# data-mermaid/mermaid-classifier

Measured on AMD Instinct MI355X. Metric: patches/sec (224x224 EfficientNet-B0), higher is better.
Workload: dtype f16; 1 GPU; EfficientNet-B0 forward, batch=256 random 224x224 u8 patches per GPU -> (256,1280) fp32; per_gpu_batch=256, global_batch=256, weights=synthetic seed 0, input_batches_rotated=8, lanes_per_gpu=2, parallelism=patch-sharded x1

## Files before the change

### mermaid_classifier_amd/csrc/k_mid.hip

```cpp
#include "device_common.h"

template <int CKS, int KSD, int CE>
__global__ __launch_bounds__(512) void mid14_kernel(Mid14Args a)
{
    constexpr int HW = 196, CH = 96, NCHK = CE / CH, NPF = 13, NTILE = 6 * NPF, NBAND = 5;
    constexpr int ES2 = 416;
    constexpr int R = KSD / 2, NP = KSD == 5 ? 3 : 2;
    static_assert(CE % CH == 0, "chunking");
    extern __shared__ __attribute__((aligned(16))) unsigned char smem[];
    constexpr int ZT = R, ZB = R + 1;
    unsigned char* E = smem + ZT * 7 * ES2;
    float* pband = reinterpret_cast<float*>(smem + (98 + 7 * (ZT + ZB)) * ES2);
    const int tid = threadIdx.x, lane = tid & 63, wave = __builtin_amdgcn_readfirstlane(tid >> 6);
    const int m = lane & 15, q = lane >> 4;
    const int b = blockIdx.x;
    const int Cin = a.Cin;
    const GLOBAL_AS _Float16* wexp = sgpr_ptr<_Float16>(a.wexp);
    const GLOBAL_AS float* bexp = sgpr_ptr<float>(a.bexp);
    const GLOBAL_AS uint32_t* dwp = sgpr_ptr<uint32_t>(a.dwp);
    const GLOBAL_AS float* bdw = sgpr_ptr<float>(a.bdw);
    const int npf = wave < 5 ? 2 : 1;
    const int pf0 = wave < 5 ? 2 * wave : wave + 5;
    const GLOBAL_AS _Float16* xgp = sgpr_ptr<_Float16>(a.X) + (size_t)b * HW * Cin;
    const int band0 = tid / CH, cd = tid - band0 * CH;
// ... 72 lines not shown
#pragma unroll
                        for (int i = 0; i < NPFW; ++i) acc[i] = __builtin_amdgcn_mfma_f32_16x16x32_f16(xb[i][ks], wc[ks], acc[i], 0, 0, 0);
                    float t[4 * NPFW];
#pragma unroll
                    for (int i = 0; i < NPFW; ++i)
#pragma unroll
                        for (int j = 0; j < 4; ++j) t[4 * i + j] = acc[i][j];
                    silu_scaled_staged(t);
#pragma unroll
                    for (int i = 0; i < NPFW; ++i) {
                        const int pix0 = 16 * (pf0 + i) + 4 * q;
                        const h2 p0 = {(_Float16)t[4 * i], (_Float16)t[4 * i + 1]};
                        const h2 p1 = {(_Float16)t[4 * i + 2], (_Float16)t[4 * i + 3]};
                        const bool ok = pix0 < HW;
                        unsigned char* dst = E + (pix0 >> 1) * ES2 + (16 * nf + m) * 4;
                        *reinterpret_cast<h2*>(ok ? dst : scratch) = p0;
                        *reinterpret_cast<h2*>(ok ? dst + ES2 : scratch + 256) = p1;
                    }
                }
            };
            if (npf == 2) expand_chunk(std::integral_constant<int, 2>{});
            else expand_chunk(std::integral_constant<int, 1>{});
        }
        T7_BAR();
        {
            constexpr int NR = 3 + 2 * R;
            const unsigned char* col = E + 4 * cd + ((rb - R) * 7) * ES2;
            uint32_t P[NR][7];
#pragma unroll
            for (int r = 0; r < NR; ++r)
#pragma unroll
                for (int pp = 0; pp < 7; ++pp) P[r][pp] = *reinterpret_cast<const uint32_t*>(col + (r * 7 + pp) * ES2);
            f2 psum2 = {0.f, 0.f};
            uint16_t* dg = reinterpret_cast<uint16_t*>(a.D + (size_t)b * HW * CE + chunk * CH + cd);
#pragma unroll
            for (int ro = 0; ro < 3; ++ro) {
                const int oy = rb + ro;
                if (oy < 14) {
                    float acc[14];
                    bool started[14] = {false, false, false, false, false, false, false, false, false, false, false, false, false, false};
#pragma unroll
                    for (int ky = 0; ky < KSD; ++ky) {
                        const uint32_t r0 = raw[3 * ky], r1 = raw[3 * ky + 1], r2 = raw[3 * ky + 2];
                        uint32_t wq[2][3];
                        if (KSD == 5) {
                            wq[0][0] = r0; wq[0][1] = r1; wq[0][2] = r2;
                            wq[1][0] = r0 << 16; wq[1][1] = __builtin_amdgcn_alignbit(r1, r0, 16); wq[1][2] = __builtin_amdgcn_alignbit(r2, r1, 16);
                        } else {
                            wq[0][0] = r0 << 16; wq[0][1] = __builtin_amdgcn_alignbit(r1, r0, 16); wq[0][2] = 0u;
                            wq[1][0] = r0; wq[1][1] = r1; wq[1][2] = 0u;
                        }
#pragma unroll
                        for (int ip = 0; ip < NP; ++ip)
#pragma unroll
                            for (int ox = 0; ox < 14; ++ox) {
                                const int fp = (KSD == 5 || !(ox & 1)) ? (ox >> 1) - 1 : (ox >> 1);
                                const int xpc = fp + ip;
                                if (xpc < 0 || xpc > 6) continue;
                                if (!started[ox]) { acc[ox] = dot2_from(P[ro + ky][xpc], wq[ox & 1][ip], dbias); started[ox] = true; }
                                else acc[ox] = __builtin_amdgcn_fdot2(*reinterpret_cast<const h2*>(&P[ro + ky][xpc]),
                                                                      *reinterpret_cast<const h2*>(&wq[ox & 1][ip]), acc[ox], false);
                            }
                    }
                    silu_scaled_staged(acc);
#pragma unroll
                    for (int ox = 0; ox < 14; ox += 2) {
                        const f2 v = {acc[ox], acc[ox + 1]};
                        psum2 = psum2 + v;
                        const uint32_t hv = cvt_pk_f16(acc[ox], acc[ox + 1]);
                        dg[(size_t)(oy * 14 + ox) * CE] = (uint16_t)hv;
                        dg[(size_t)(oy * 14 + ox + 1) * CE] = (uint16_t)(hv >> 16);
                    }
                }
            }
            pband[band * CH + cd] = (psum2.x + psum2.y) + 0.f;
        }
        T7_BAR();
        if (tid < CH)
            a.pool[(size_t)b * CE + chunk * CH + tid] =
                ((pband[tid] + pband[CH + tid]) + pband[2 * CH + tid]) + pband[3 * CH + tid] + pband[4 * CH + tid];
    }
}

template <int CKS, int KSD, int CE>
__global__ __launch_bounds__(512) void mid14m_kernel(Mid14Args a)
{
    constexpr int HW = 196, NG = CE / 16, R = KSD / 2;
    constexpr int XSTR = 64 * CKS + 16;
    constexpr int ERS = 40;
    constexpr int ECS = 736;
    constexpr int EREG = 16 * ECS;
    constexpr int TREG = 56 * 32;
    extern __shared__ __attribute__((aligned(16))) unsigned char smem[];
    unsigned char* XS = smem;
    const int tid = threadIdx.x, lane = tid & 63, wave = __builtin_amdgcn_readfirstlane(tid >> 6);
    unsigned char* EW = smem + HW * XSTR + wave * (EREG + TREG);
    unsigned char* TW = EW + EREG;
    const int n16 = lane & 15, q = lane >> 4;
    const int blk = lane >> 2, n = lane & 3;
    const int c = 2 * (blk & 3) + ((blk >> 2) & 1) + 8 * (blk >> 3);
    const int b = blockIdx.x;
    const int Cin = a.Cin;
    const GLOBAL_AS _Float16* wexp = sgpr_ptr<_Float16>(a.wexp);
    const GLOBAL_AS float* bexp = sgpr_ptr<float>(a.bexp);
    const GLOBAL_AS _Float16* dwt = sgpr_ptr<_Float16>(a.dwdiag);
    const GLOBAL_AS float* bdw = sgpr_ptr<float>(a.bdw);
    const bool clk = a.dbg_clk != nullptr;
    long long ck[5] = {clk ? (long long)__builtin_readcyclecounter() : 0, 0, 0, 0, 0};
    {
        const _Float16* xg = a.X + (size_t)b * HW * Cin;
        constexpr int CPR = 4 * CKS;
        constexpr int NIT = (HW * CPR + 511) / 512;
        uint4 xv[NIT];
        for (int e = lane; e < EREG / 16; e += 64) *reinterpret_cast<uint4*>(EW + 16 * e) = uint4{0u, 0u, 0u, 0u};
#pragma unroll
        for (int it = 0; it < NIT; ++it) {
            const int e0 = tid + 512 * it, e = e0 < HW * CPR ? e0 : HW * CPR - 1;
            const int row = e / CPR, cc = e - row * CPR;
            xv[it] = *reinterpret_cast<const uint4*>(xg + (size_t)row * Cin + (8 * cc < Cin ? 8 * cc : Cin - 8));
        }
#pragma unroll
        for (int it = 0; it < NIT; ++it) {
            const int e = tid + 512 * it;
            const int row = e / CPR, cc = e - row * CPR;
            const uint4 v = 8 * cc < Cin ? xv[it] : uint4{0u, 0u, 0u, 0u};
            if (e < HW * CPR) *reinterpret_cast<uint4*>(XS + row * XSTR + 16 * cc) = v;
        }
    }
    __syncthreads();
    if (clk) ck[1] = (long long)__builtin_readcyclecounter();
    const unsigned char* xrow = XS + (n16 < 14 ? n16 : 13) * XSTR + 16 * q;
    unsigned char* est = EW + n16 * ECS + 2 * ERS + 8 * q;
    const uint32_t m3 = q == 3 ? 0u : 0xffffffffu;
    const unsigned char* dld = EW + c * ECS + n * ERS + (2 - R) * ERS;
    const unsigned char* dld3 = EW + c * ECS + (n < 2 ? n : 1) * ERS + (2 - R) * ERS;
    unsigned char* tst = TW + (n * 14 + (((blk >> 2) & 1) ? 7 : 0)) * 32 + (c >> 1) * 4;
    h8 we[CKS], wen[CKS];
    u2v ta[KSD][2], tan[KSD][2];
    float be, bd, ben, bdn;
    auto request_group = [&](int g, h8 (&w1)[CKS], u2v (&w2)[KSD][2], float& b1, float& b2) {
#pragma unroll
        for (int ks = 0; ks < CKS; ++ks) w1[ks] = gload<h8>(wexp, (unsigned)(((g * CKS + ks) * 64 + lane) * 16));
        b1 = gload<float>(bexp, (unsigned)(16 * g + n16) * 4u);
#pragma unroll
        for (int ky = 0; ky < KSD; ++ky)
#pragma unroll
            for (int h = 0; h < 2; ++h) w2[ky][h] = gload<u2v>(dwt, (unsigned)((((g * KSD + ky) * 2 + h) * 64 + lane) * 8));
        b2 = gload<float>(bdw, (unsigned)(16 * g + c) * 4u);
    };
    {
        const int g0 = blockIdx.y * 8 + wave;
        request_group(g0 < NG ? g0 : 0, wen, tan, ben, bdn);
    }
#pragma unroll 1
    for (int g = blockIdx.y * 8 + wave; g < NG; g += 8 * gridDim.y) {
#pragma unroll
        for (int ks = 0; ks < CKS; ++ks) we[ks] = wen[ks];
#pragma unroll
        for (int ky = 0; ky < KSD; ++ky) { ta[ky][0] = tan[ky][0]; ta[ky][1] = tan[ky][1]; }
        be = ben;
        bd = bdn;
        {
            const int gn = g + 8 * (int)gridDim.y;
            request_group(gn < NG ? gn : g, wen, tan, ben, bdn);
        }
        PIN_VMEM();
        auto x_frags = [&](int y, h8 (&xb)[2][CKS]) {
#pragma unroll
            for (int u = 0; u < 2; ++u)
#pragma unroll
                for (int ks = 0; ks < CKS; ++ks) xb[u][ks] = *reinterpret_cast<const h8*>(xrow + (y + u) * 14 * XSTR + 64 * ks);
        };
        auto x_epilogue = [&](int y, const f4 (&acc)[2]) {
            float t[8] = {acc[0][0], acc[0][1], acc[0][2], acc[0][3], acc[1][0], acc[1][1], acc[1][2], acc[1][3]};
            silu_scaled_staged(t);
#pragma unroll
            for (int u = 0; u < 2; ++u) {
                const u2v o = {cvt_pk_f16(t[4 * u], t[4 * u + 1]), cvt_pk_f16(t[4 * u + 2], t[4 * u + 3]) & m3};
                *reinterpret_cast<u2v*>(est + (y + u) * ERS) = o;
            }
        };
        {
            const f4 bev = {be, be, be, be};
            h8 xf[2][2][CKS];
            f4 accp[2] = {bev, bev};
            x_frags(0, xf[0]);
#pragma unroll
            for (int st = 0; st < 7; ++st) {
                if (st + 1 < 7) x_frags(2 * (st + 1), xf[(st + 1) & 1]);
                __builtin_amdgcn_sched_barrier(0);
                f4 acc[2];
#pragma unroll
                for (int ks = 0; ks < CKS; ++ks)
#pragma unroll
                    for (int u = 0; u < 2; ++u)
                        acc[u] = __builtin_amdgcn_mfma_f32_16x16x32_f16(xf[st & 1][u][ks], we[ks], ks == 0 ? bev : acc[u], 0, 0, 0);
                if (st > 0) x_epilogue(2 * (st - 1), accp);
                if (st > 0) {
#pragma unroll
                    for (int i = 0; i < 2 * CKS; ++i) {
                        __builtin_amdgcn_sched_group_barrier(0x008, 1, 0);
                        __builtin_amdgcn_sched_group_barrier(0x002, 5, 0);
                    }
                }
                __builtin_amdgcn_sched_barrier(0);
#pragma unroll
                for (int u = 0; u < 2; ++u) accp[u] = acc[u];
            }
            x_epilogue(12, accp);
        }
        if (clk && ck[2] == 0) ck[2] = (long long)__builtin_readcyclecounter();
        float psum = 0.f;
        unsigned char* dgb = reinterpret_cast<unsigned char*>(a.D + (size_t)b * HW * CE + 16 * g);
        auto d_quads = [&](auto yt_tag, h4 (&bq)[KSD][4]) {
            constexpr int YT = decltype(yt_tag)::value;
            const unsigned char* rb = YT == 3 ? dld3 : dld;
#pragma unroll
            for (int ky = 0; ky < KSD; ++ky)
#pragma unroll
                for (int x4 = 0; x4 < 4; ++x4) bq[ky][x4] = *reinterpret_cast<const h4*>(rb + (4 * YT + ky) * ERS + 8 * x4);
        };
        auto d_strip = [&](const h4 (&bq)[KSD][4], f4 (&acc)[4]) {
            const f4 bdv = {bd, bd, bd, bd};
#pragma unroll
            for (int ky = 0; ky < KSD; ++ky) {
                const h4 a0 = __builtin_bit_cast(h4, ta[ky][0]), a1 = __builtin_bit_cast(h4, ta[ky][1]);
#pragma unroll
                for (int xt = 0; xt < 4; ++xt) acc[xt] = __builtin_amdgcn_mfma_f32_4x4x4f16(a1, bq[ky][xt], ky == 0 ? bdv : acc[xt], 0, 0, 0);
#pragma unroll
                for (int xt = 1; xt < 4; ++xt) acc[xt] = __builtin_amdgcn_mfma_f32_4x4x4f16(a0, bq[ky][xt - 1], acc[xt], 0, 0, 0);
            }
        };
        auto d_epilogue = [&](auto yt_tag, const f4 (&acc)[4]) {
            constexpr int YT = decltype(yt_tag)::value;
            float v[14];
#pragma unroll
            for (int x = 0; x < 14; ++x) v[x] = acc[(x + 2) >> 2][(x + 2) & 3];
            silu_scaled_staged(v);
            float s = ((v[0] + v[1]) + (v[2] + v[3])) + ((v[4] + v[5]) + (v[6] + v[7])) + ((v[8] + v[9]) + (v[10] + v[11])) + (v[12] + v[13]);
            if (YT == 3) s = n < 2 ? s : 0.f;
            psum += s;
#ifdef MID14M_NOSWAP
#pragma unroll
            for (int x = 0; x < 14; x += 2) {
                const uint32_t hv = cvt_pk_f16(v[x], v[x + 1]);
                *reinterpret_cast<uint16_t*>(TW + (n * 14 + x) * 32 + c * 2) = (uint16_t)hv;
                *reinterpret_cast<uint16_t*>(TW + (n * 14 + x + 1) * 32 + c * 2) = (uint16_t)(hv >> 16);
            }
#else
#pragma unroll
            for (int j = 0; j < 7; ++j) {
                float lo = v[j], hi = v[7 + j];
                asm volatile("s_nop 1\n\tv_permlane16_swap_b32 %0, %1\n\ts_nop 1" : "+v"(lo), "+v"(hi));
                *reinterpret_cast<uint32_t*>(tst + j * 32) = cvt_pk_f16(lo, hi);
            }
#endif
            constexpr int NV = YT == 3 ? 56 : 112;
#pragma unroll
            for (int r = 0; r < 2; ++r) {
                if (64 * r >= NV) break;
                const int v0 = lane + 64 * r, vi = v0 < NV ? v0 : NV - 1;
                const uint4 o = *reinterpret_cast<const uint4*>(TW + vi * 16);
                *reinterpret_cast<uint4*>(dgb + (size_t)(56 * YT + (vi >> 1)) * (CE * 2) + 16 * (vi & 1)) = o;
            }
        };
        {
            using I0 = std::integral_constant<int, 0>; using I1 = std::integral_constant<int, 1>;
            using I2 = std::integral_constant<int, 2>; using I3 = std::integral_constant<int, 3>;
            h4 bqa[KSD][4], bqb[KSD][4];
            f4 acc0[4], acc1[4];
            d_quads(I0{}, bqa);
            d_quads(I1{}, bqb);
            __builtin_amdgcn_sched_barrier(0);
            d_strip(bqa, acc0);
            __builtin_amdgcn_sched_barrier(0);
            d_quads(I2{}, bqa);
            __builtin_amdgcn_sched_barrier(0);
            d_strip(bqb, acc1);
            d_epilogue(I0{}, acc0);
            __builtin_amdgcn_sched_barrier(0);
            d_quads(I3{}, bqb);
            __builtin_amdgcn_sched_barrier(0);
            d_strip(bqa, acc0);
            d_epilogue(I1{}, acc1);
            __builtin_amdgcn_sched_barrier(0);
            d_strip(bqb, acc1);
            d_epilogue(I2{}, acc0);
            __builtin_amdgcn_sched_barrier(0);
            d_epilogue(I3{}, acc1);
        }
        psum = quad_sum(psum);
        if (n == 0) a.pool[(size_t)b * CE + 16 * g + c] = psum;
        if (clk && ck[3] == 0) ck[3] = (long long)__builtin_readcyclecounter();
    }
    if (clk && lane == 0 && (wave == 0 || wave == 4 || wave == 7)) {
        ck[4] = (long long)__builtin_readcyclecounter();
        float* dst = a.dbg_clk + ((size_t)b * 8 + blockIdx.y) * 16 + (wave == 0 ? 0 : (wave == 4 ? 4 : 8));
        dst[0] = (float)(ck[1] - ck[0]); dst[1] = (float)(ck[2] - ck[1]); dst[2] = (float)(ck[3] - ck[2]); dst[3] = (float)(ck[4] - ck[3]);
    }
}

template <int KS, int NF, int HW, bool RES>
__global__ __launch_bounds__(512) void proj_patch_kernel(ProjPatchArgs a)
{
    constexpr int CK = (KS <= 8) ? KS : (KS % 7 == 0 ? 3 : (KS % 5 == 0 ? (NF <= 5 ? 3 : 5) : 6));
    constexpr int NCH = KS / CK;
    static_assert(KS % CK == 0, "chunking");
    constexpr int NPF = (HW + 15) / 16, NPAIR = (NPF + 1) / 2;
    constexpr int NWCH = NF * KS * 64;
    constexpr int WPT = (NWCH + 511) / 512;
    constexpr int KP = 32 * KS;
    constexpr bool EARLY_RES = KS < 21;
    extern __shared__ __attribute__((aligned(16))) unsigned char smem[];
    unsigned char* wl = smem;
    float* pooled = reinterpret_cast<float*>(smem + NF * KS * 1024);
    float* gate = pooled + KP;
    float* rs = gate + KP;
    const int tid = threadIdx.x, lane = tid & 63, wave = __builtin_amdgcn_readfirstlane(tid >> 6);
    const int m = lane & 15, q = lane >> 4;
    const int b = blockIdx.x;
    const int K = a.K, CSP = a.CSP;
    long long tk0 = 0, tk1 = 0, tk2 = 0;
    if (a.dbg_clk) tk0 = (long long)__builtin_readcyclecounter();
    const GLOBAL_AS _Float16* wfrag = sgpr_ptr<_Float16>(a.wfrag);
    const GLOBAL_AS _Float16* wr_g = sgpr_ptr<_Float16>(a.wr_g);
    const GLOBAL_AS _Float16* we_t = sgpr_ptr<_Float16>(a.we_t);
    const GLOBAL_AS float* pp = sgpr_ptr<float>(a.pool_part);
    constexpr int FC1_IT = (KP + 63) / 64, KPAD = 64 * FC1_IT;
    const int G = CSP >> 2;
    const bool fc1_wave = wave < G;
    const GLOBAL_AS _Float16* xg = sgpr_ptr<_Float16>(a.X) + (size_t)b * HW * K;
    auto load_chunk = [&](int pr, int ch, h8 (&dst)[2][CK]) {
#pragma unroll
        for (int i = 0; i < 2; ++i) {
            const int p = 32 * pr + 16 * i + m;
            const int pix = p < HW ? p : HW - 1;
#pragma unroll
            for (int u = 0; u < CK; ++u) {
                const int k = 32 * (ch * CK + u) + 8 * q;
                dst[i][u] = gload<h8>(xg, (unsigned)((pix * K + (k < K ? k : K - 8)) * 2));
            }
        }
    };
    constexpr int NW = NF * KS;
    constexpr int DS0 = NW < 44 ? NW : 44, DS1 = NW - DS0 < 50 ? NW - DS0 : 50;
    auto dma = [&](auto i0_tag, auto i1_tag) {
        constexpr int I0 = decltype(i0_tag)::value, I1 = decltype(i1_tag)::value;
#pragma unroll
        for (int i = I0; i < I1; ++i)
            __builtin_amdgcn_global_load_lds((const __attribute__((address_space(1))) void*)(a.wfrag + ((size_t)i * 64 + lane) * 8),
                                             (__attribute__((address_space(3))) void*)(wl + i * 1024), 16, 0, 0);
        PIN_VMEM();
    };
    h8 xc[2][CK], xn[2][CK];
    f4 bv[NF];
    const GLOBAL_AS float* biasg = sgpr_ptr<float>(a.bias);
    auto load_bias = [&]() {
#pragma unroll
        for (int nf = 0; nf < NF; ++nf) bv[nf] = gload<f4>(biasg, (unsigned)(16 * nf + 4 * q) * 4u);
    };
    if (wave == 7) {
        __builtin_amdgcn_s_barrier();
        dma(std::integral_constant<int, 0>{}, std::integral_constant<int, DS0>{});
        T7_BAR();
        dma(std::integral_constant<int, DS0>{}, std::integral_constant<int, DS0 + DS1>{});
        T7_BAR();
        dma(std::integral_constant<int, DS0 + DS1>{}, std::integral_constant<int, NW>{});
        load_bias();
        if (7 < NPAIR) { load_chunk(7, 0, xc); PIN_VMEM(); }
        asm volatile("s_waitcnt vmcnt(0)" ::: "memory");
        T7_BAR();
    } else {
        static_assert(KP <= 672, "channel 448..511 reassignment assumes no channel t + 512 for t >= 160");
        float ps0 = 0.f, ps1 = 0.f;
        const int pk0 = tid, pk1 = (tid >= 160 && tid < 224) ? tid + 288 : tid + 512;
        {
            const int k0 = pk0 < K ? pk0 : 0, k1 = pk1 < K ? pk1 : 0;
            if (a.nparts == 1) {
                ps0 = gload<float>(pp, (unsigned)((b * K + k0) * 4));
                ps1 = gload<float>(pp, (unsigned)((b * K + k1) * 4));
            } else {
                float v0[16], v1[16];
#pragma unroll
                for (int p = 0; p < 16; ++p) {
                    const int pc = p < a.nparts ? p : 0;
                    v0[p] = gload<float>(pp, (unsigned)(((b * a.nparts + pc) * K + k0) * 4));
                    v1[p] = gload<float>(pp, (unsigned)(((b * a.nparts + pc) * K + k1) * 4));
                }
#pragma unroll
                for (int p = 0; p < 16; ++p) {
                    ps0 += p < a.nparts ? v0[p] : 0.f;
                    ps1 += p < a.nparts ? v1[p] : 0.f;
                }
            }
        }
        const int wj = fc1_wave ? wave : 0;
        u2v w1[FC1_IT];
#pragma unroll
        for (int i = 0; i < FC1_IT; ++i) w1[i] = gload<u2v>(wr_g, (unsigned)(((wj * KPAD + lane + 64 * i) * 4) * 2));
        const int k2 = 2 * tid;
        const bool fc2_thr = k2 < K;
        uint32_t w2[28];
#pragma unroll
        for (int j = 0; j < 28; ++j) w2[j] = gload<uint32_t>(we_t, (unsigned)(((j < CSP ? j : 0) * K + (fc2_thr ? k2 : 0)) * 2));
        const float be0 = fc2_thr ? a.be[k2] : 0.f, be1 = fc2_thr ? a.be[k2 + 1] : 0.f;
        load_bias();
        const float brv = a.br[4 * wj + (lane & 3)];
    PIN_VMEM();
    __builtin_amdgcn_s_barrier();
    if (pk0 < KP) pooled[pk0] = pk0 < K ? ps0 : 0.f;
    if (pk1 < KP) pooled[pk1] = pk1 < K ? ps1 : 0.f;
    T7_BAR();
    if (a.dbg_clk && tid == 0) a.dbg_clk[(size_t)b * 8 + 3] = (float)((long long)__builtin_readcyclecounter() - tk0);
    if (fc1_wave) {
        float xs[FC1_IT];
#pragma unroll
        for (int i = 0; i < FC1_IT; ++i) {
            const int k = lane + 64 * i;
            xs[i] = pooled[k < KP ? k : 0];
        }
        __builtin_amdgcn_sched_barrier(0);
        float acc[4] = {0.f, 0.f, 0.f, 0.f};
#pragma unroll
        for (int i = 0; i < FC1_IT; ++i) {
            acc[0] = fma_mix_lo(w1[i].x, xs[i], acc[0]);
            acc[1] = fma_mix_hi(w1[i].x, xs[i], acc[1]);
            acc[2] = fma_mix_lo(w1[i].y, xs[i], acc[2]);
            acc[3] = fma_mix_hi(w1[i].y, xs[i], acc[3]);
        }
        float tot[4];
#pragma unroll
        for (int j = 0; j < 4; ++j) {
            const int v = __builtin_bit_cast(int, row16_sum(acc[j]));
            tot[j] = (__builtin_bit_cast(float, __builtin_amdgcn_readlane(v, 0)) + __builtin_bit_cast(float, __builtin_amdgcn_readlane(v, 16))) +
                     (__builtin_bit_cast(float, __builtin_amdgcn_readlane(v, 32)) + __builtin_bit_cast(float, __builtin_amdgcn_readlane(v, 48)));
        }
        if (lane < 4) {
            const float sv = lane == 0 ? tot[0] : (lane == 1 ? tot[1] : (lane == 2 ? tot[2] : tot[3]));
            rs[4 * wave + lane] = silu_f(sv * a.psc + brv);
        }
    }
    T7_BAR();
    if (a.dbg_clk && tid == 0) {
        a.dbg_clk[(size_t)b * 8 + 4] = (float)((long long)__builtin_readcyclecounter() - tk0);
        a.dbg_clk[(size_t)b * 8 + 5] = a.dbg_clk[(size_t)b * 8 + 4];
    }
    static_assert(NPAIR >= 7, "waves 0..6 all own a pair of pixel fragments");
    load_chunk(wave, 0, xc);
    PIN_VMEM();
    if (k2 < KP) {
        float a0 = be0, a1 = be1;
// ... 200 lines not shown
```

### mermaid_classifier_amd/csrc/k_tail.hip

```cpp
#include "device_common.h"

#define T7_PIX 49
#define T7_C 192
#define T7_CE 1152
#define T7_XS 400
#define T7_ES 2320
#define T7_YS 656
#define T7_DS11 1552
#define T7_OFF_X (T7_PIX * T7_ES)
#define T7_OFF_POOL (T7_OFF_X + T7_PIX * T7_XS)
#define T7_OFF_RS (T7_OFF_POOL + T7_CE * 4)
#define T7_OFF_GATE (T7_OFF_RS + 48 * 4)
#define T7_OFF_PART (T7_OFF_GATE + T7_CE * 4)
#define T7_LDS 163680
static_assert(T7_LDS >= T7_OFF_PART + 32 * 48 * 4 && T7_LDS <= 163840, "tail7 LDS map");

#ifndef T7_GATE_IN_WEIGHTS
#define T7_GATE_IN_WEIGHTS 0
#endif

#define DW_SILU(acc) silu_scaled_staged(acc)
__global__ __launch_bounds__(512) void tail7_kernel(TailArgs a)
{
    extern __shared__ __attribute__((aligned(16))) unsigned char smem[];
// ... 6 lines not shown
    const int tid0 = threadIdx.x;
    const int b = blockIdx.x;
    const bool clk_on = a.dbg_clk && a.clk_sections;
    long long tkk[6] = {0, 0, 0, 0, 0, 0};
    if (clk_on) tkk[0] = (long long)__builtin_readcyclecounter();
    auto proj_prefetch = [&](const GLOBAL_AS _Float16* wproj, const GLOBAL_AS float* bproj, int KS, int nf0, int nfn, int lane, int q,
                             f4 (&pbias)[3], unsigned (&wo)[3], h8 (&wa)[3][4]) {
#pragma unroll
        for (int i = 0; i < 3; ++i) {
            const int nf = nf0 + (i < nfn ? i : 0);
            pbias[i] = gload<f4>(bproj, (unsigned)(16 * nf + 4 * q) * 4u);
            wo[i] = (unsigned)((nf * KS * 64 + lane) * 16);
#pragma unroll
            for (int d = 0; d < 4; ++d) wa[i][d] = gload<h8>(wproj, wo[i] + (unsigned)(d * 1024));
        }
    };
    auto proj_run = [&](const GLOBAL_AS _Float16* wproj, int KS, int mode, int nf0, int nfn, int lane, int m, int q,
                        const int (&pixc)[4], f4 (&pbias)[3], unsigned (&wo)[3], h8 (&wa)[3][4], int es = T7_ES) {
        f4 acc[3][4];
#pragma unroll
        for (int i = 0; i < 3; ++i)
#pragma unroll
            for (int pf = 0; pf < 4; ++pf) acc[i][pf] = pbias[i];
        const unsigned char* bxp[4];
#pragma unroll
        for (int pf = 0; pf < 4; ++pf) bxp[pf] = ED + pixc[pf] * es + 16 * q;
        auto k_loop = [&](auto nf_tag, auto ks_tag) {
            constexpr int NF = decltype(nf_tag)::value, KSC = decltype(ks_tag)::value;
            static_assert(KSC % 4 == 0 && KSC >= 8, "k-steps come in sets of four");
            h8 bx[4], bn[4], wb[NF][4];
#pragma unroll
            for (int pf = 0; pf < 4; ++pf) bx[pf] = *reinterpret_cast<const h8*>(bxp[pf]);
            f4 gc0 = *reinterpret_cast<const f4*>(gate + 8 * q), gc1 = *reinterpret_cast<const f4*>(gate + 8 * q + 4), gn0, gn1;
            auto gated = [&](const h8& w) -> h8 {
                if (!T7_GATE_IN_WEIGHTS) return w;
                const uint4 o = gate_h8(*reinterpret_cast<const uint4*>(&w), gc0, gc1);
                return *reinterpret_cast<const h8*>(&o);
            };
            auto step = [&](int ks, const h8 (&wset)[3][4], int d) {
                const int kn = ks + 1 < KSC ? ks + 1 : KSC - 1;
#pragma unroll
                for (int pf = 0; pf < 4; ++pf) bn[pf] = *reinterpret_cast<const h8*>(bxp[pf] + 64 * kn);
                if (T7_GATE_IN_WEIGHTS) {
                    gn0 = *reinterpret_cast<const f4*>(gate + 32 * kn + 8 * q);
                    gn1 = *reinterpret_cast<const f4*>(gate + 32 * kn + 8 * q + 4);
                }
                h8 wg[NF];
#pragma unroll
                for (int i = 0; i < NF; ++i) wg[i] = gated(wset[i][d]);
#pragma unroll
                for (int i = 0; i < NF; ++i)
#pragma unroll
                    for (int pf = 0; pf < 4; ++pf)
                        acc[i][pf] = __builtin_amdgcn_mfma_f32_16x16x32_f16(wg[i], bx[pf], acc[i][pf], 0, 0, 0);
#pragma unroll
                for (int pf = 0; pf < 4; ++pf) bx[pf] = bn[pf];
                gc0 = gn0; gc1 = gn1;
            };
            auto stepb = [&](int ks, int d) {
                const int kn = ks + 1 < KSC ? ks + 1 : KSC - 1;
#pragma unroll
                for (int pf = 0; pf < 4; ++pf) bn[pf] = *reinterpret_cast<const h8*>(bxp[pf] + 64 * kn);
                if (T7_GATE_IN_WEIGHTS) {
                    gn0 = *reinterpret_cast<const f4*>(gate + 32 * kn + 8 * q);
                    gn1 = *reinterpret_cast<const f4*>(gate + 32 * kn + 8 * q + 4);
                }
                h8 wg[NF];
#pragma unroll
                for (int i = 0; i < NF; ++i) wg[i] = gated(wb[i][d]);
#pragma unroll
                for (int i = 0; i < NF; ++i)
#pragma unroll
                    for (int pf = 0; pf < 4; ++pf)
                        acc[i][pf] = __builtin_amdgcn_mfma_f32_16x16x32_f16(wg[i], bx[pf], acc[i][pf], 0, 0, 0);
#pragma unroll
                for (int pf = 0; pf < 4; ++pf) bx[pf] = bn[pf];
                gc0 = gn0; gc1 = gn1;
            };
#pragma unroll 1
            for (int k0 = 0; k0 + 8 <= KSC; k0 += 8) {
#pragma unroll
                for (int d = 0; d < 4; ++d) {
#pragma unroll
                    for (int i = 0; i < NF; ++i) wb[i][d] = gload<h8>(wproj, wo[i] + (unsigned)((k0 + 4 + d) * 1024));
                    PIN_VMEM();
                    step(k0 + d, wa, d);
                    PIN_VMEM();
                }
#pragma unroll
                for (int d = 0; d < 4; ++d) {
                    const int kw = k0 + 8 + d < KSC ? k0 + 8 + d : KSC - 1;
#pragma unroll
                    for (int i = 0; i < NF; ++i) wa[i][d] = gload<h8>(wproj, wo[i] + (unsigned)(kw * 1024));
                    PIN_VMEM();
                    stepb(k0 + 4 + d, d);
                    PIN_VMEM();
                }
            }
            if (KSC % 8) {
#pragma unroll
                for (int d = 0; d < 4; ++d) step(KSC - 4 + d, wa, d);
            }
        };
        auto run_nf = [&](auto ks_tag) {
            if (nfn == 3) k_loop(std::integral_constant<int, 3>{}, ks_tag);
            else if (nfn == 2) k_loop(std::integral_constant<int, 2>{}, ks_tag);
            else k_loop(std::integral_constant<int, 1>{}, ks_tag);
        };
        if (KS == 36) run_nf(std::integral_constant<int, 36>{});
        else run_nf(std::integral_constant<int, 24>{});
        if (mode == 1) {
            T7_BAR();
#pragma unroll
            for (int pf = 0; pf < 4; ++pf) {
                if (16 * pf + m >= T7_PIX) continue;
#pragma unroll
                for (int i = 0; i < 3; ++i) {
                    if (i >= nfn) continue;
                    h4 o;
#pragma unroll
                    for (int j = 0; j < 4; ++j) o[j] = (_Float16)acc[i][pf][j];
                    *reinterpret_cast<h4*>(ED + (16 * pf + m) * T7_YS + (16 * (nf0 + i) + 4 * q) * 2) = o;
                }
            }
        } else {
#pragma unroll
            for (int pf = 0; pf < 4; ++pf) {
                if (16 * pf + m >= T7_PIX) continue;
#pragma unroll
                for (int i = 0; i < 2; ++i) {
                    if (i >= nfn) continue;
                    h4* px = reinterpret_cast<h4*>(XL + (16 * pf + m) * T7_XS + (16 * (nf0 + i) + 4 * q) * 2);
                    h4 r = {0, 0, 0, 0};
                    if (mode == 0) r = *px;
                    h4 o;
#pragma unroll
                    for (int j = 0; j < 4; ++j) o[j] = (_Float16)(acc[i][pf][j] + (float)r[j]);
                    *px = o;
                }
            }
        }
    };
    if (a.pre_D || a.pre_X) {
        const int DS = a.pre_X ? T7_DS11 : T7_ES;
        const int tid = tid0, lane = tid & 63, wave = __builtin_amdgcn_readfirstlane(tid >> 6);
        const int m = lane & 15, q = lane >> 4;
        const GLOBAL_AS _Float16* wr_t = sgpr_ptr<_Float16>(a.pre_wr_t);
        const GLOBAL_AS _Float16* we_t = sgpr_ptr<_Float16>(a.pre_we_t);
        const GLOBAL_AS _Float16* wproj = sgpr_ptr<_Float16>(a.pre_wproj);
        const GLOBAL_AS float* bproj = sgpr_ptr<float>(a.pre_bproj);
        const int sl = tid / 7, j4 = tid - sl * 7;
        const bool fc_thr = tid < 336;
        u2v w1[14];
#pragma unroll
        for (int i = 0; i < 14; ++i) w1[i] = gload<u2v>(wr_t, (unsigned)((((fc_thr ? sl : 0) + 48 * i) * 28 + 4 * j4) * 2));
        uint32_t w2[28];
#pragma unroll
        for (int j = 0; j < 28; ++j) w2[j] = gload<uint32_t>(we_t, (unsigned)((j * 672 + (fc_thr ? 2 * tid : 0)) * 2));
        const float be0 = fc_thr ? a.pre_be[2 * tid] : 0.f, be1 = fc_thr ? a.pre_be[2 * tid + 1] : 0.f;
        const float brv = tid < 28 ? a.pre_br[tid] : 0.f;
        if (a.pre_X) {
            constexpr int CH = 96, ES2 = 416;
            unsigned char* EB = ED + T7_PIX * T7_DS11 + 7 * ES2;
            float* pband = part;
            const GLOBAL_AS _Float16* wexp = sgpr_ptr<_Float16>(a.pre_wexp);
            const GLOBAL_AS float* bexp = sgpr_ptr<float>(a.pre_bexp);
            const GLOBAL_AS uint32_t* dwp = sgpr_ptr<uint32_t>(a.pre_dwp);
            const GLOBAL_AS float* bdw = sgpr_ptr<float>(a.pre_bdw);
            const GLOBAL_AS _Float16* xgp = sgpr_ptr<_Float16>(a.pre_X) + (size_t)b * 196 * 112;
            const int npf = wave < 5 ? 2 : 1;
            const int pf0 = wave < 5 ? 2 * wave : wave + 5;
            h8 xb[2][4];
#pragma unroll
            for (int i = 0; i < 2; ++i) {
                const int pix = 16 * (pf0 + (i < npf ? i : 0)) + m;
                const int pixc = pix < 196 ? pix : 195;
#pragma unroll
                for (int ks = 0; ks < 4; ++ks) {
                    const int kk = 32 * ks + 8 * q;
                    xb[i][ks] = gload<h8>(xgp, (unsigned)((pixc * 112 + (kk < 112 ? kk : 104)) * 2));
                }
            }
            for (int e = tid; e < T7_PIX * 12; e += 512) {
                const int pix = e / 12, oc = e - pix * 12;
                *reinterpret_cast<uint4*>(ED + pix * T7_DS11 + 1344 + oc * 16) = uint4{0u, 0u, 0u, 0u};
            }
            for (int e = tid; e < 35 * (ES2 / 16); e += 512) {
                const int row = e / (ES2 / 16), c16 = e - row * (ES2 / 16);
                *reinterpret_cast<uint4*>(EB + (row < 7 ? row - 7 : row + 91) * ES2 + 16 * c16) = uint4{0u, 0u, 0u, 0u};
            }
            const int band = tid / CH, cd = tid - band * CH;
            h8 wn[4];
            float bsn = gload<float>(bexp, (unsigned)m * 4u);
#pragma unroll
            for (int ks = 0; ks < 4; ++ks) wn[ks] = gload<h8>(wexp, (unsigned)((ks * 64 + lane) * 16));
            unsigned char* const scratch = reinterpret_cast<unsigned char*>(part) + 3072 + lane * 4;
            auto expand_chunk = [&](auto npf_tag, int chunk) {
                constexpr int NPF = decltype(npf_tag)::value;
#pragma unroll
                for (int nf = 0; nf < 6; ++nf) {
                    const int nfg = 6 * chunk + nf;
                    h8 wc[4];
#pragma unroll
                    for (int ks = 0; ks < 4; ++ks) wc[ks] = wn[ks];
                    const float bs = bsn;
                    {
                        const int nxt = nfg + 1 < 42 ? nfg + 1 : 41;
                        bsn = gload<float>(bexp, (unsigned)(16 * nxt + m) * 4u);
#pragma unroll
                        for (int ks = 0; ks < 4; ++ks) wn[ks] = gload<h8>(wexp, (unsigned)(((nxt * 4 + ks) * 64 + lane) * 16));
                    }
                    PIN_VMEM();
                    const f4 bv = {bs, bs, bs, bs};
                    f4 acc[NPF];
#pragma unroll
                    for (int i = 0; i < NPF; ++i) acc[i] = bv;
#pragma unroll
                    for (int ks = 0; ks < 4; ++ks)
#pragma unroll
                        for (int i = 0; i < NPF; ++i) acc[i] = __builtin_amdgcn_mfma_f32_16x16x32_f16(xb[i][ks], wc[ks], acc[i], 0, 0, 0);
                    float t[4 * NPF];
#pragma unroll
                    for (int i = 0; i < NPF; ++i)
#pragma unroll
                        for (int j = 0; j < 4; ++j) t[4 * i + j] = acc[i][j];
                    silu_scaled_staged(t);
#pragma unroll
                    for (int i = 0; i < NPF; ++i) {
                        const int pix0 = 16 * (pf0 + i) + 4 * q;
                        const h2 p0 = {(_Float16)t[4 * i], (_Float16)t[4 * i + 1]};
                        const h2 p1 = {(_Float16)t[4 * i + 2], (_Float16)t[4 * i + 3]};
                        const bool ok = pix0 < 196;
                        unsigned char* dst = EB + (pix0 >> 1) * ES2 + (16 * nf + m) * 4;
                        *reinterpret_cast<h2*>(ok ? dst : scratch) = p0;
                        *reinterpret_cast<h2*>(ok ? dst + ES2 : scratch + 256) = p1;
                    }
                }
            };
#pragma unroll 1
            for (int chunk = 0; chunk < 7; ++chunk) {
                uint32_t raw[15];
                const int cg = chunk * CH + cd;
#pragma unroll
                for (int i = 0; i < 15; ++i) raw[i] = 0u;
                float dbias;
                {
                    u4v t4[4];
#pragma unroll
                    for (int j = 0; j < 4; ++j) t4[j] = gload<u4v>(dwp, (unsigned)((j * 672 + cg) * 16));
#pragma unroll
                    for (int j = 0; j < 4; ++j) {
                        raw[4 * j] = t4[j].x; raw[4 * j + 1] = t4[j].y; raw[4 * j + 2] = t4[j].z;
                        if (j < 3) raw[4 * j + 3] = t4[j].w;
                    }
                    dbias = __builtin_bit_cast(float, (uint32_t)t4[3].w);
                }
                if (npf == 2) expand_chunk(std::integral_constant<int, 2>{}, chunk);
                else expand_chunk(std::integral_constant<int, 1>{}, chunk);
                T7_BAR();
#pragma unroll 1
                for (int pass = 0; pass < 2; ++pass) {
                    if (pass == 1 && wave >= 3) break;
                    const int oy = pass == 0 ? band : (band == 0 ? 6 : 5);
                    const unsigned char* col = EB + 4 * cd + ((2 * oy - 1) * 7) * ES2;
                    uint32_t P[5][7];
#pragma unroll
                    for (int r = 0; r < 5; ++r)
#pragma unroll
                        for (int pp = 0; pp < 7; ++pp) P[r][pp] = *reinterpret_cast<const uint32_t*>(col + (r * 7 + pp) * ES2);
                    unsigned char* dcol = ED + (chunk * CH + cd) * 2;
                    float acc[7];
                    bool started[7] = {false, false, false, false, false, false, false};
#pragma unroll
                    for (int ky = 0; ky < 5; ++ky) {
                        const uint32_t r0 = raw[3 * ky], r1 = raw[3 * ky + 1], r2 = raw[3 * ky + 2];
                        const uint32_t wq[3] = {r0 << 16, __builtin_amdgcn_alignbit(r1, r0, 16), __builtin_amdgcn_alignbit(r2, r1, 16)};
#pragma unroll
                        for (int ip = 0; ip < 3; ++ip)
#pragma unroll
                            for (int ox = 0; ox < 7; ++ox) {
                                const int xpc = ox - 1 + ip;
                                if (xpc < 0 || xpc > 6) continue;
                                if (!started[ox]) { acc[ox] = dot2_from(P[ky][xpc], wq[ip], dbias); started[ox] = true; }
                                else acc[ox] = __builtin_amdgcn_fdot2(*reinterpret_cast<const h2*>(&P[ky][xpc]),
                                                                      *reinterpret_cast<const h2*>(&wq[ip]), acc[ox], false);
                            }
                    }
                    silu_scaled_staged(acc);
                    f2 psum2 = {0.f, 0.f};
#pragma unroll
                    for (int ox = 0; ox < 6; ox += 2) {
                        const f2 v = {acc[ox], acc[ox + 1]};
                        psum2 = psum2 + v;
                        const uint32_t hv = cvt_pk_f16(acc[ox], acc[ox + 1]);
                        *reinterpret_cast<uint16_t*>(dcol + (oy * 7 + ox) * T7_DS11) = (uint16_t)hv;
                        *reinterpret_cast<uint16_t*>(dcol + (oy * 7 + ox + 1) * T7_DS11) = (uint16_t)(hv >> 16);
                    }
                    *reinterpret_cast<_Float16*>(dcol + (oy * 7 + 6) * T7_DS11) = (_Float16)acc[6];
                    pband[oy * CH + cd] = (psum2.x + psum2.y) + acc[6];
                }
                T7_BAR();
                if (tid < CH)
                    pooled[chunk * CH + tid] = (((pband[tid] + pband[CH + tid]) + (pband[2 * CH + tid] + pband[3 * CH + tid])) +
                                                (pband[4 * CH + tid] + pband[5 * CH + tid])) + pband[6 * CH + tid];
            }
            if (a.dbg_dw) {
                T7_BAR();
                for (int e = tid; e < T7_PIX * 84; e += 512) {
                    const int pix = e / 84, oc = e - pix * 84;
                    *reinterpret_cast<uint4*>(a.dbg_dw + ((size_t)b * T7_PIX + pix) * 672 + oc * 8) = *reinterpret_cast<const uint4*>(ED + pix * T7_DS11 + oc * 16);
                }
            }
        } else {
            const _Float16* dg = a.pre_D + (size_t)b * T7_PIX * 672;
            for (int e = tid; e < T7_PIX * 96; e += 512) {
                const int pix = e / 96, oc = e - pix * 96;
                h8 v = {0, 0, 0, 0, 0, 0, 0, 0};
                if (oc < 84) v = *reinterpret_cast<const h8*>(dg + pix * 672 + oc * 8);
                *reinterpret_cast<h8*>(ED + pix * T7_ES + oc * 16) = v;
            }
            for (int kk = tid; kk < 672; kk += 512) pooled[kk] = a.pre_pool[(size_t)b * 672 + kk];
        }
        T7_BAR();
        if (clk_on) tkk[1] = (long long)__builtin_readcyclecounter();
        if (fc_thr) {
            f4 acc = {0.f, 0.f, 0.f, 0.f};
#pragma unroll
            for (int i = 0; i < 14; ++i) {
                const float x = pooled[sl + 48 * i];
                acc[0] = fma_mix_lo(w1[i].x, x, acc[0]);
                acc[1] = fma_mix_hi(w1[i].x, x, acc[1]);
                acc[2] = fma_mix_lo(w1[i].y, x, acc[2]);
                acc[3] = fma_mix_hi(w1[i].y, x, acc[3]);
            }
            *reinterpret_cast<f4*>(part + sl * 32 + 4 * j4) = acc;
        }
        T7_BAR();
        if (tid < 28) {
            float s = 0.f;
#pragma unroll
            for (int w0 = 0; w0 < 48; w0 += 16) {
                float pv[16];
#pragma unroll
                for (int w = 0; w < 16; ++w) pv[w] = part[(w0 + w) * 32 + tid];
#pragma unroll
                for (int w = 0; w < 16; ++w) s += pv[w];
            }
            rs[tid] = silu_f(s * (float)(1.0 / (49.0 * 1.4426950408889634)) + brv);
        }
        T7_BAR();
        {
            float a0 = be0, a1 = be1;
#pragma unroll
            for (int j = 0; j < 28; ++j) {
                const float r = rs[j];
                a0 = fma_mix_lo(w2[j], r, a0);
                a1 = fma_mix_hi(w2[j], r, a1);
            }
            if (fc_thr) {
                const float g0 = sigmoid_f(a0), g1 = sigmoid_f(a1);
                gate[2 * tid] = g0;
                gate[2 * tid + 1] = g1;
                if (a.dbg_gate) {
                    a.dbg_gate[(size_t)b * 672 + 2 * tid] = g0;
                    a.dbg_gate[(size_t)b * 672 + 2 * tid + 1] = g1;
                }
            }
        }
        const bool lowh = wave < 4;
        const int nfn = lowh ? 2 : 1, nf0 = lowh ? 2 * wave : wave + 4;
        int pixc[4];
#pragma unroll
        for (int pf = 0; pf < 4; ++pf) pixc[pf] = (16 * pf + m) < T7_PIX ? (16 * pf + m) : (T7_PIX - 1);
        f4 pbias[3];
        unsigned wo[3];
        h8 wa[3][4];
        proj_prefetch(wproj, bproj, 24, nf0, nfn, lane, q, pbias, wo, wa);
        T7_BAR();
        if (clk_on) tkk[2] = (long long)__builtin_readcyclecounter();
        if (T7_GATE_IN_WEIGHTS) {
            if (tid < 96) gate[672 + tid] = 0.f;
        } else
        if (tid < 504) {
            const int r6 = tid / 84, oc = tid - 84 * r6;
            const f4 g0 = *reinterpret_cast<const f4*>(gate + oc * 8);
            const f4 g1 = *reinterpret_cast<const f4*>(gate + oc * 8 + 4);
            unsigned char* pc = ED + oc * 16;
            for (int k0 = 0; k0 < 9; k0 += 3) {
                uint4 v[3];
#pragma unroll
                for (int j = 0; j < 3; ++j) {
                    const int pix = r6 + 6 * (k0 + j);
                    v[j] = *reinterpret_cast<const uint4*>(pc + (pix < T7_PIX ? pix : T7_PIX - 1) * DS);
                }
#pragma unroll
                for (int j = 0; j < 3; ++j) {
                    const int pix = r6 + 6 * (k0 + j);
                    const uint4 o = gate_h8(v[j], g0, g1);
                    if (pix < T7_PIX) *reinterpret_cast<uint4*>(pc + pix * DS) = o;
                }
            }
        }
        T7_BAR();
        if (clk_on) tkk[3] = (long long)__builtin_readcyclecounter();
        proj_run(wproj, 24, 2, nf0, nfn, lane, m, q, pixc, pbias, wo, wa, DS);
        T7_BAR();
        if (clk_on) {
            tkk[4] = (long long)__builtin_readcyclecounter();
            if (tid0 == 0) for (int i = 0; i < 4; ++i) a.dbg_clk[((size_t)b * 8) * 8 + i] = (float)(tkk[i + 1] - tkk[i]);
        }
    } else if (a.in_wide) {
        const int tid = tid0;
        const _Float16* xg = a.X + (size_t)b * T7_PIX * 320;
        for (int e = tid; e < T7_PIX * 40; e += 512) {
            const int pix = e / 40, p16 = e - pix * 40;
            *reinterpret_cast<h8*>(ED + pix * T7_YS + p16 * 16) = *reinterpret_cast<const h8*>(xg + pix * 320 + p16 * 8);
        }
        __syncthreads();
    } else {
        const int tid = tid0;
        const _Float16* xg = a.X + (size_t)b * T7_PIX * T7_C;
        for (int e = tid; e < T7_PIX * 24; e += 512) {
            const int pix = e / 24, p16 = e - pix * 24;
            *reinterpret_cast<h8*>(XL + pix * T7_XS + p16 * 16) = *reinterpret_cast<const h8*>(xg + pix * T7_C + p16 * 8);
        }
        __syncthreads();
    }
    bool out_wide = a.in_wide != 0;
#pragma unroll 1
    for (int nb = 0; nb < a.nblk; ++nb) {
        const TailBlock Wt = a.blk[nb];
        struct {
            const GLOBAL_AS _Float16* wexp; const GLOBAL_AS float* bexp; const GLOBAL_AS uint32_t* dwp; const GLOBAL_AS float* bdw;
            const GLOBAL_AS _Float16* wr_t; const GLOBAL_AS float* br; const GLOBAL_AS _Float16* we_t; const GLOBAL_AS float* be;
            const GLOBAL_AS _Float16* wproj; const GLOBAL_AS float* bproj;
        } W = {sgpr_ptr<_Float16>(Wt.wexp), sgpr_ptr<float>(Wt.bexp), sgpr_ptr<uint32_t>(Wt.dwp), sgpr_ptr<float>(Wt.bdw),
               sgpr_ptr<_Float16>(Wt.wr_t), sgpr_ptr<float>(Wt.br), sgpr_ptr<_Float16>(Wt.we_t), sgpr_ptr<float>(Wt.be),
               sgpr_ptr<_Float16>(Wt.wproj), sgpr_ptr<float>(Wt.bproj)};
        int tid = tid0;
        asm volatile("" : "+v"(tid));
        const int lane = tid & 63, wave = __builtin_amdgcn_readfirstlane(tid >> 6);
        const int m = lane & 15, q = lane >> 4;
        long long tk[7];
        int ntk = 0;
#define T7_TICK() do { if (a.dbg_clk) tk[ntk] = (long long)__builtin_readcyclecounter(); ++ntk; } while (0)
        T7_TICK();
        int pixc[4];
#pragma unroll
        for (int pf = 0; pf < 4; ++pf) pixc[pf] = (16 * pf + m) < T7_PIX ? (16 * pf + m) : (T7_PIX - 1);
        const bool ks3 = Wt.ks == 3;
        uint32_t rawA[15], rawB[15];
        float biasA, biasB;
        auto load_taps = [&](int ch, uint32_t (&raw)[15], float& bias) {
            u4v t4[4];
#pragma unroll
            for (int j = 0; j < 4; ++j) t4[j] = gload<u4v>(W.dwp, (unsigned)((j * T7_CE + ch) * 16));
#pragma unroll
            for (int j = 0; j < 4; ++j) {
                raw[4 * j] = t4[j].x; raw[4 * j + 1] = t4[j].y; raw[4 * j + 2] = t4[j].z;
                if (j < 3) raw[4 * j + 3] = t4[j].w;
            }
            bias = __builtin_bit_cast(float, (uint32_t)t4[3].w);
        };
        load_taps(tid, rawA, biasA);
        {
            h8 xb[4][6];
// ... 455 lines not shown
```

Before: 235,400 patches/s.

## Rebalance tail7 fused expand work per wave and defer FC weight loads

In the fused pre-stage of tail7, the expand 1x1 conv now splits its work across waves as (pixel-fragment, channel-pair) items from lookup tables, so each wave computes 5 items with two weight fragments each, instead of looping over all 6 channel groups for 1 or 2 pixel fragments. MFMA for one item is interleaved with the SiLU/store epilogue of the previous item using sched_group_barrier. Weight loads for the next chunk are issued after the current chunk's expand, and the FC weight register loads are moved to after the depthwise loop, which cuts register pressure during the main loop. Cycle-counter instrumentation is also added to both kernels. It adds more register state (xb[5][4] plus two weight sets) and a table-driven mapping that is hard to follow.

```diff
diff --git a/mermaid_classifier_amd/csrc/k_mid.hip b/mermaid_classifier_amd/csrc/k_mid.hip
--- a/mermaid_classifier_amd/csrc/k_mid.hip
+++ b/mermaid_classifier_amd/csrc/k_mid.hip
@@ -248,8 +248,10 @@
         const int g0 = blockIdx.y * 8 + wave;
         request_group(g0 < NG ? g0 : 0, wen, tan, ben, bdn);
     }
+    long long ckl = 0;
 #pragma unroll 1
     for (int g = blockIdx.y * 8 + wave; g < NG; g += 8 * gridDim.y) {
+        if (clk && g >= NG / 8 * 8) ckl = (long long)__builtin_readcyclecounter();
 #pragma unroll
         for (int ks = 0; ks < CKS; ++ks) we[ks] = wen[ks];
 #pragma unroll
@@ -393,6 +395,7 @@
         ck[4] = (long long)__builtin_readcyclecounter();
         float* dst = a.dbg_clk + ((size_t)b * 8 + blockIdx.y) * 16 + (wave == 0 ? 0 : (wave == 4 ? 4 : 8));
         dst[0] = (float)(ck[1] - ck[0]); dst[1] = (float)(ck[2] - ck[1]); dst[2] = (float)(ck[3] - ck[2]); dst[3] = (float)(ck[4] - ck[3]);
+        a.dbg_clk[((size_t)b * 8 + blockIdx.y) * 16 + 12 + (wave == 0 ? 0 : (wave == 4 ? 1 : 2))] = ckl ? (float)(ck[4] - ckl) : 0.f;
     }
 }
 
diff --git a/mermaid_classifier_amd/csrc/k_tail.hip b/mermaid_classifier_amd/csrc/k_tail.hip
--- a/mermaid_classifier_amd/csrc/k_tail.hip
+++ b/mermaid_classifier_amd/csrc/k_tail.hip
@@ -182,13 +182,18 @@
         const int sl = tid / 7, j4 = tid - sl * 7;
         const bool fc_thr = tid < 336;
         u2v w1[14];
-#pragma unroll
-        for (int i = 0; i < 14; ++i) w1[i] = gload<u2v>(wr_t, (unsigned)((((fc_thr ? sl : 0) + 48 * i) * 28 + 4 * j4) * 2));
         uint32_t w2[28];
-#pragma unroll
-        for (int j = 0; j < 28; ++j) w2[j] = gload<uint32_t>(we_t, (unsigned)((j * 672 + (fc_thr ? 2 * tid : 0)) * 2));
-        const float be0 = fc_thr ? a.pre_be[2 * tid] : 0.f, be1 = fc_thr ? a.pre_be[2 * tid + 1] : 0.f;
-        const float brv = tid < 28 ? a.pre_br[tid] : 0.f;
+        float be0, be1, brv;
+        auto request_fc = [&](int t) {
+            const int slt = t / 7, j4t = t - slt * 7;
+            const bool thr = t < 336;
+#pragma unroll
+            for (int i = 0; i < 14; ++i) w1[i] = gload<u2v>(wr_t, (unsigned)((((thr ? slt : 0) + 48 * i) * 28 + 4 * j4t) * 2));
+#pragma unroll
+            for (int j = 0; j < 28; ++j) w2[j] = gload<uint32_t>(we_t, (unsigned)((j * 672 + (thr ? 2 * t : 0)) * 2));
+            be0 = thr ? a.pre_be[2 * t] : 0.f; be1 = thr ? a.pre_be[2 * t + 1] : 0.f;
+            brv = t < 28 ? a.pre_br[t] : 0.f;
+        };
         if (a.pre_X) {
             constexpr int CH = 96, ES2 = 416;
             unsigned char* EB = ED + T7_PIX * T7_DS11 + 7 * ES2;
@@ -198,12 +203,13 @@
             const GLOBAL_AS uint32_t* dwp = sgpr_ptr<uint32_t>(a.pre_dwp);
             const GLOBAL_AS float* bdw = sgpr_ptr<float>(a.pre_bdw);
             const GLOBAL_AS _Float16* xgp = sgpr_ptr<_Float16>(a.pre_X) + (size_t)b * 196 * 112;
-            const int npf = wave < 5 ? 2 : 1;
-            const int pf0 = wave < 5 ? 2 * wave : wave + 5;
-            h8 xb[2][4];
-#pragma unroll
-            for (int i = 0; i < 2; ++i) {
-                const int pix = 16 * (pf0 + (i < npf ? i : 0)) + m;
+            const int prA = (0x22111000u >> (4 * wave)) & 15, prB = (0x22200211u >> (4 * wave)) & 15;
+            const int pfA = (0x30630630u >> (4 * wave)) & 15, pfB = (0xCA8B96B9u >> (4 * wave)) & 15;
+            int ipf[5] = {pfA, pfA + 1, pfA + 2, pfB, pfB < 12 ? pfB + 1 : 12};
+            h8 xb[5][4];
+#pragma unroll
+            for (int i = 0; i < 5; ++i) {
+                const int pix = 16 * ipf[i] + m;
                 const int pixc = pix < 196 ? pix : 195;
 #pragma unroll
                 for (int ks = 0; ks < 4; ++ks) {
@@ -220,53 +226,72 @@
                 *reinterpret_cast<uint4*>(EB + (row < 7 ? row - 7 : row + 91) * ES2 + 16 * c16) = uint4{0u, 0u, 0u, 0u};
             }
             const int band = tid / CH, cd = tid - band * CH;
-            h8 wn[4];
-            float bsn = gload<float>(bexp, (unsigned)m * 4u);
-#pragma unroll
-            for (int ks = 0; ks < 4; ++ks) wn[ks] = gload<h8>(wexp, (unsigned)((ks * 64 + lane) * 16));
+            h8 wA[2][4], wB[2][4];
+            float bsA[2], bsB[2];
+            auto request_pairs = [&](int chunk) {
+#pragma unroll
+                for (int j = 0; j < 2; ++j) {
+                    bsA[j] = gload<float>(bexp, (unsigned)(16 * (6 * chunk + 2 * prA + j) + m) * 4u);
+                    bsB[j] = gload<float>(bexp, (unsigned)(16 * (6 * chunk + 2 * prB + j) + m) * 4u);
+                }
+#pragma unroll
+                for (int j = 0; j < 2; ++j)
+#pragma unroll
+                    for (int ks = 0; ks < 4; ++ks) wA[j][ks] = gload<h8>(wexp, (unsigned)((((6 * chunk + 2 * prA + j) * 4 + ks) * 64 + lane) * 16));
+#pragma unroll
+                for (int j = 0; j < 2; ++j)
+#pragma unroll
+                    for (int ks = 0; ks < 4; ++ks) wB[j][ks] = gload<h8>(wexp, (unsigned)((((6 * chunk + 2 * prB + j) * 4 + ks) * 64 + lane) * 16));
+            };
+            request_pairs(0);
             unsigned char* const scratch = reinterpret_cast<unsigned char*>(part) + 3072 + lane * 4;
-            auto expand_chunk = [&](auto npf_tag, int chunk) {
-                constexpr int NPF = decltype(npf_tag)::value;
-#pragma unroll
-                for (int nf = 0; nf < 6; ++nf) {
-                    const int nfg = 6 * chunk + nf;
-                    h8 wc[4];
-#pragma unroll
-                    for (int ks = 0; ks < 4; ++ks) wc[ks] = wn[ks];
-                    const float bs = bsn;
-                    {
-                        const int nxt = nfg + 1 < 42 ? nfg + 1 : 41;
-                        bsn = gload<float>(bexp, (unsigned)(16 * nxt + m) * 4u);
-#pragma unroll
-                        for (int ks = 0; ks < 4; ++ks) wn[ks] = gload<h8>(wexp, (unsigned)(((nxt * 4 + ks) * 64 + lane) * 16));
-                    }
-                    PIN_VMEM();
-                    const f4 bv = {bs, bs, bs, bs};
-                    f4 acc[NPF];
-#pragma unroll
-                    for (int i = 0; i < NPF; ++i) acc[i] = bv;
-#pragma unroll
-                    for (int ks = 0; ks < 4; ++ks)
-#pragma unroll
-                        for (int i = 0; i < NPF; ++i) acc[i] = __builtin_amdgcn_mfma_f32_16x16x32_f16(xb[i][ks], wc[ks], acc[i], 0, 0, 0);
-                    float t[4 * NPF];
-#pragma unroll
-                    for (int i = 0; i < NPF; ++i)
-#pragma unroll
-                        for (int j = 0; j < 4; ++j) t[4 * i + j] = acc[i][j];
-                    silu_scaled_staged(t);
-#pragma unroll
-                    for (int i = 0; i < NPF; ++i) {
-                        const int pix0 = 16 * (pf0 + i) + 4 * q;
-                        const h2 p0 = {(_Float16)t[4 * i], (_Float16)t[4 * i + 1]};
-                        const h2 p1 = {(_Float16)t[4 * i + 2], (_Float16)t[4 * i + 3]};
-                        const bool ok = pix0 < 196;
-                        unsigned char* dst = EB + (pix0 >> 1) * ES2 + (16 * nf + m) * 4;
-                        *reinterpret_cast<h2*>(ok ? dst : scratch) = p0;
-                        *reinterpret_cast<h2*>(ok ? dst + ES2 : scratch + 256) = p1;
-                    }
-                }
+            auto item_mfma = [&](const h8 (&xi)[4], const h8 (&w)[2][4], const float (&bs)[2], f4 (&acc)[2]) {
+#pragma unroll
+                for (int j = 0; j < 2; ++j) acc[j] = f4{bs[j], bs[j], bs[j], bs[j]};
+#pragma unroll
+                for (int ks = 0; ks < 4; ++ks)
+#pragma unroll
+                    for (int j = 0; j < 2; ++j) acc[j] = __builtin_amdgcn_mfma_f32_16x16x32_f16(xi[ks], w[j][ks], acc[j], 0, 0, 0);
             };
+            auto item_epilogue = [&](int pf, int pr, const f4 (&acc)[2]) {
+                float t[8] = {acc[0][0], acc[0][1], acc[0][2], acc[0][3], acc[1][0], acc[1][1], acc[1][2], acc[1][3]};
+                silu_scaled_staged(t);
+                const int pix0 = 16 * pf + 4 * q;
+                const bool ok = pix0 < 196;
+                unsigned char* dst = EB + (pix0 >> 1) * ES2 + (32 * pr + m) * 4;
+#pragma unroll
+                for (int j = 0; j < 2; ++j) {
+                    const h2 p0 = {(_Float16)t[4 * j], (_Float16)t[4 * j + 1]};
+                    const h2 p1 = {(_Float16)t[4 * j + 2], (_Float16)t[4 * j + 3]};
+                    *reinterpret_cast<h2*>(ok ? dst + 64 * j : scratch) = p0;
+                    *reinterpret_cast<h2*>(ok ? dst + 64 * j + ES2 : scratch + 256) = p1;
+                }
+            };
+            auto expand_chunk = [&]() {
+                f4 accp[2];
+#pragma unroll
+                for (int i = 0; i < 5; ++i) {
+                    f4 acc[2];
+                    __builtin_amdgcn_sched_barrier(0);
+                    if (i < 3) item_mfma(xb[i], wA, bsA, acc);
+                    else item_mfma(xb[i], wB, bsB, acc);
+                    if (i > 0) {
+                        item_epilogue(ipf[i - 1], i - 1 < 3 ? prA : prB, accp);
+#pragma unroll
+                        for (int u = 0; u < 8; ++u) {
+                            __builtin_amdgcn_sched_group_barrier(0x008, 1, 0);
+                            __builtin_amdgcn_sched_group_barrier(0x002, 5, 0);
+                        }
+                    }
+                    __builtin_amdgcn_sched_barrier(0);
+#pragma unroll
+                    for (int j = 0; j < 2; ++j) accp[j] = acc[j];
+                }
+                item_epilogue(ipf[4], prB, accp);
+            };
+            long long tsub[4] = {0, 0, 0, 0}, tprol = 0, tc = 0;
+            if (clk_on) { tc = (long long)__builtin_readcyclecounter(); tprol = tc - tkk[0]; }
+#define T7_SUB(i) do { if (clk_on) { const long long now__ = (long long)__builtin_readcyclecounter(); tsub[i] += now__ - tc; tc = now__; } } while (0)
 #pragma unroll 1
             for (int chunk = 0; chunk < 7; ++chunk) {
                 uint32_t raw[15];
@@ -285,9 +310,12 @@
                     }
                     dbias = __builtin_bit_cast(float, (uint32_t)t4[3].w);
                 }
-                if (npf == 2) expand_chunk(std::integral_constant<int, 2>{}, chunk);
-                else expand_chunk(std::integral_constant<int, 1>{}, chunk);
+                expand_chunk();
+                request_pairs(chunk < 6 ? chunk + 1 : 6);
+                PIN_VMEM();
+                T7_SUB(0);
                 T7_BAR();
+                T7_SUB(3);
 #pragma unroll 1
                 for (int pass = 0; pass < 2; ++pass) {
                     if (pass == 1 && wave >= 3) break;
@@ -328,11 +356,25 @@
                     }
                     *reinterpret_cast<_Float16*>(dcol + (oy * 7 + 6) * T7_DS11) = (_Float16)acc[6];
                     pband[oy * CH + cd] = (psum2.x + psum2.y) + acc[6];
+                    if (pass == 0) T7_SUB(1); else T7_SUB(2);
                 }
                 T7_BAR();
+                T7_SUB(3);
                 if (tid < CH)
                     pooled[chunk * CH + tid] = (((pband[tid] + pband[CH + tid]) + (pband[2 * CH + tid] + pband[3 * CH + tid])) +
                                                 (pband[4 * CH + tid] + pband[5 * CH + tid])) + pband[6 * CH + tid];
+            }
+#undef T7_SUB
+            {
+                int tf = tid;
+                asm volatile("" : "+v"(tf));
+                request_fc(tf);
+            }
+            PIN_VMEM();
+            if (clk_on && tid0 == 0) {
+                float* dst = a.dbg_clk + ((size_t)b * 8 + 7) * 8;
+                dst[0] = (float)tprol;
+                for (int i = 0; i < 4; ++i) dst[1 + i] = (float)tsub[i];
             }
             if (a.dbg_dw) {
                 T7_BAR();
@@ -342,6 +384,7 @@
                 }
             }
         } else {
+            request_fc(tid);
             const _Float16* dg = a.pre_D + (size_t)b * T7_PIX * 672;
             for (int e = tid; e < T7_PIX * 96; e += 512) {
                 const int pix = e / 96, oc = e - pix * 96;
```

Result: no change. 236,100 patches/s (median of 6 runs) (+0.3%).
